# AdrienCorenflos/aux-ssm-samplers

Measured on AMD Instinct MI355X. Metric: Gibbs sweeps/sec (aux-Kalman, parallel-in-time scan), higher is better.
Workload: dtype f64; 1 GPU; C2: linear-Gaussian SSM T=65536 d=4 p=8, aux-Kalman sweep, parallel scan; chains_per_gpu=256, parallelism=chains x1 (independent, no collective)

## Files before the change

### aux_ssm_samplers_amd/csrc/fused_shared.h

```cpp
#pragma once

struct FusedArgs {
    int C, T, E, nchunk;
    const void* xa;
    void* xb;
    const int32_t* sel;
    void* u;
    void* inc;
    const void* gain;
    const void* samp;
    const void* logt;
    const void* gpre;
    const void* m0p;
    void* agg_f; void* pre_f; void* agg_s; void* pre_s;
    Acc* pa;
    Acc* pe;
    void* pell;
    const Acc* clog;
    const int* nanrow;
    unsigned ka0, ka1, ks0, ks1;
    const void* eps0s;
    double delta, shd;
    const double* dptr;
    int nan_policy;
// ... 191 lines not shown
                    sample_offset<R, D>(G[q], acc, e[h + q], o);
#pragma unroll
                    for (int i = 0; i < D; ++i) acc[i] = j == j0 ? e[h + q][i] : o[i];
                }
            }
        }
    }
    R Gs[DD];
    ldmat(gks, 0, Gs);
#pragma unroll
    for (int s = 0; s < FS_MID_STAGES; ++s) {
        const int off = 1 << s;
        R Gn[DD];
        ldmat(gks, s + 1 < FS_MID_STAGES ? s + 1 : s, Gn);
        stv<R, D>(lds + tid * Pre::NPAD, acc);
        __syncthreads();
        R left[D];
        ldv<R, D>(lds + max(tid - off, 0) * Pre::NPAD, left);
        __syncthreads();
        R o[D];
        sample_offset<R, D>(Gs, left, acc, o);
#pragma unroll
        for (int i = 0; i < D; ++i) acc[i] = tid >= off ? o[i] : acc[i];
#pragma unroll
        for (int k = 0; k < DD; ++k) Gs[k] = Gn[k];
    }
    stv<R, D>(lds + tid * Pre::NPAD, acc);
    __syncthreads();
    R p[D];
    ldv<R, D>(lds + max(tid - 1, 0) * Pre::NPAD, p);
#pragma unroll
    for (int i = 0; i < D; ++i) p[i] = tid > 0 ? p[i] : (R)0;
    for (int jb = j0; jb < j1; jb += NR) {
        if (E2 > NR) load_block(jb);
#pragma unroll
        for (int h = 0; h < NR; h += NG) {
            R G[NG][DD];
#pragma unroll
            for (int q = 0; q < NG; ++q) ldmat(gser, min(jb + h + q, jlast) - j0, G[q]);
#pragma unroll
            for (int q = 0; q < NG; ++q) {
                const int j = jb + h + q;
                if (j < j1) {
                    stv<R, D>(pre + (long long)j * Pre::NPAD, p);
                    R o[D];
                    sample_offset<R, D>(G[q], p, e[h + q], o);
#pragma unroll
                    for (int i = 0; i < D; ++i) p[i] = o[i];
                }
            }
        }
    }
}
template <typename R, int D>
__global__ void __launch_bounds__(TB_AGGS) k_fs_mid(FusedArgs a, const R* __restrict__ gtab_f, const R* __restrict__ gtab_s) {
    using Pre = SampPre<R, D>;
    __shared__ __attribute__((aligned(16))) R lds[TB_AGGS * Pre::NPAD];
    const long long base = (long long)blockIdx.x * a.nchunk * Pre::NPAD;
    R* pre_f = (R*)a.pre_f + base;
    const size_t nks = fs_mid_ks_reals<D>(), nser = fs_mid_ser_reals<D>(a.nchunk);
    fs_mid_scan<R, D, false>(lds, a.nchunk, (const R*)a.agg_f + base, pre_f, gtab_f, gtab_f + nks, nullptr, nullptr);
    __syncthreads();
    fs_mid_scan<R, D, true>(lds, a.nchunk, (const R*)a.agg_s + base, (R*)a.pre_s + base, gtab_s, gtab_s + nks, gtab_s + nks + nser, pre_f);
}

template <typename R, int D, int PO> struct FsRows {
    static constexpr int P = D + PO;
    using TL = LogShared<R, D, PO>;
    static constexpr int VEC = 16 / sizeof(R);
    static constexpr int pad(int n) { return (n + VEC - 1) / VEC * VEC; }
    static constexpr int cM = 0, cKc = D * D, cK = cKc + D, cM1 = cK + D * D, cGb = cM1 + D * D, cL = cGb + D, cGp = cL + symsize(D), cLg = cGp + D * D,
                         NC = pad(cLg + TL::N);
    static constexpr int eG = 0, eN = D * D, eL = 2 * D * D, NE = pad(eL + TL::N);
};
struct FsSrc { int tab, off; };
template <typename R, int D, int PO> __device__ __forceinline__ FsSrc fs_src_c(int k) {
    constexpr int P = D + PO;
    using F = FsRows<R, D, PO>; using TG = GainRow<R, D, P>; using TS = SampShared<R, D>; using TL = LogShared<R, D, PO>;
    if (k < F::cKc) return {0, TG::oM + k};
    if (k < F::cK) return {0, TG::oKc + (k - F::cKc)};
    if (k < F::cM1) { const int q = k - F::cK; return {0, TG::oK + (q / D) * P + (q % D)}; }
    if (k < F::cGb) return {1, TS::oM + (k - F::cM1)};
    if (k < F::cL) return {1, TS::oGb + (k - F::cGb)};
    if (k < F::cGp) {
        const int q = k - F::cL;
        int i = 0;
        while (lidx(i + 1, 0) <= q) ++i;
        return {1, TS::oL + i * D + (q - lidx(i, 0))};
    }
    if (k < F::cLg) return {3, k - F::cGp};
    if (k < F::cLg + TL::N) return {2, k - F::cLg};
    return {-1, 0};
}
template <typename R, int D, int PO> __device__ __forceinline__ FsSrc fs_src_e(int k) {
    using F = FsRows<R, D, PO>; using TS = SampShared<R, D>; using TL = LogShared<R, D, PO>;
    if (k < F::eN) return {1, TS::oG + k};
    if (k < F::eL) return {5, k - F::eN};
    if (k < F::eL + TL::N) return {4, k - F::eL};
    return {-1, 0};
}
template <typename R, int D, int PO> __global__ void __launch_bounds__(256) k_fs_rows(FusedArgs a, const R* __restrict__ ntab, R* __restrict__ rc, R* __restrict__ re,
                                                                                      int* __restrict__ nanrow) {
    if (memo_skip(a)) return;
    constexpr int P = D + PO;
    using F = FsRows<R, D, PO>; using TG = GainRow<R, D, P>; using TS = SampShared<R, D>; using TL = LogShared<R, D, PO>;
    const int fam = blockIdx.y;
    const int N = fam == 0 ? F::NC : F::NE;
    const long long g = (long long)blockIdx.x * 256 + threadIdx.x;
    if (g >= (long long)a.T * N) return;
    const int t = (int)(g / N), k = (int)(g % N);
    const FsSrc sc = fam == 0 ? fs_src_c<R, D, PO>(k) : fs_src_e<R, D, PO>(k);
    R v = 0;
    if (sc.tab == 0) { if (t >= 1) v = ((const R*)a.gain)[(long long)(t - 1) * TG::NPAD + sc.off]; }
    else if (sc.tab == 1) v = ((const R*)a.samp)[(long long)t * TS::NPAD + sc.off];
    else if (sc.tab == 2) { if (t >= 1) v = ((const R*)a.logt)[(long long)(t - 1) * TL::NPAD + sc.off]; }
    else if (sc.tab == 3) v = ((const R*)a.gpre)[(long long)t * D * D + sc.off];
    else if (sc.tab == 4) { if (t + 1 < a.T) v = ((const R*)a.logt)[(long long)t * TL::NPAD + sc.off]; }
    else if (sc.tab == 5) v = ntab[(long long)t * D * D + sc.off];
    (fam == 0 ? rc : re)[g] = v;
    if ((sc.tab == 2 || sc.tab == 4) && !finite_(v)) *nanrow = 1;
}

template <typename R, int D> __global__ void __launch_bounds__(256) k_fs_clog_part(int T, const R* __restrict__ samp, Acc* __restrict__ part, const int* memo) {
    if (memo_skip_p(memo)) return;
    using TS = SampShared<R, D>;
    __shared__ Acc sh[256];
    const int t = blockIdx.x * 256 + threadIdx.x;
    R s = 0;
    if (t < T) {
        const R* row = samp + (long long)t * TS::NPAD;
#pragma unroll
        for (int i = 0; i < D; ++i) s += log_(row[TS::oL + i * D + i]);
    }
    sh[threadIdx.x] = (Acc)s;
    __syncthreads();
    for (int off = 128; off > 0; off >>= 1) {
        if ((int)threadIdx.x < off) sh[threadIdx.x] += sh[threadIdx.x + off];
        __syncthreads();
    }
    if (threadIdx.x == 0) part[blockIdx.x] = sh[0];
}
template <int D> __global__ void __launch_bounds__(256) k_fs_clog_sum(int T, int nb, const Acc* __restrict__ part, Acc* __restrict__ out, int* __restrict__ nanrow,
                                                                      const int* memo) {
    if (memo_skip_p(memo)) return;
    if (threadIdx.x == 0) *nanrow = 0;
    __shared__ Acc sh[256];
    Acc acc = 0;
    for (int b = threadIdx.x; b < nb; b += 256) acc += part[b];
    sh[threadIdx.x] = acc;
    __syncthreads();
    for (int off = 128; off > 0; off >>= 1) {
        if ((int)threadIdx.x < off) sh[threadIdx.x] += sh[threadIdx.x + off];
        __syncthreads();
    }
    if (threadIdx.x == 0) *out = sh[0] + (Acc)T * (Acc)D * (Acc)(0.5 * LOG_2PI);
}

__device__ __forceinline__ void fs_block(const FusedArgs& a, int& ch, int& c, bool down = false) {
    const int groups = (a.C + (int)blockDim.x - 1) / (int)blockDim.x;
    const int q = blockIdx.x / groups;
    ch = down ? a.nchunk - 1 - q : q;
    c = (blockIdx.x % groups) * blockDim.x + threadIdx.x;
}
template <typename R, int N> __device__ __forceinline__ void fs_stage(const R* __restrict__ tab, int r0, int r1, R* __restrict__ lds) {
    using V = typename Vec16<R>::type;
    constexpr int W = Vec16<R>::W;
    const V* src = reinterpret_cast<const V*>(tab + (long long)r0 * N);
    V* dst = reinterpret_cast<V*>(lds);
    const int n = (r1 - r0) * (N / W), B = blockDim.x;
    for (int i = threadIdx.x; i < n; i += 4 * B) {
        const bool p1 = i + B < n, p2 = i + 2 * B < n, p3 = i + 3 * B < n;
        const V v0 = src[i], v1 = p1 ? src[i + B] : V{}, v2 = p2 ? src[i + 2 * B] : V{}, v3 = p3 ? src[i + 3 * B] : V{};
        dst[i] = v0;
        if (p1) dst[i + B] = v1;
        if (p2) dst[i + 2 * B] = v2;
        if (p3) dst[i + 3 * B] = v3;
    }
    __syncthreads();
}

template <typename R, int N> __device__ __forceinline__ void fs_stage_pk(const R* __restrict__ tab, int r0, int r1, int E, R* __restrict__ lds) {
    using V = typename Vec16<R>::type;
    constexpr int W = Vec16<R>::W, NV = N / W;
    const V* src = reinterpret_cast<const V*>(tab + (long long)r0 * N);
    V* dst = reinterpret_cast<V*>(lds);
    const int n = (r1 - r0) * NV, B = blockDim.x;
    for (int i = threadIdx.x; i < n; i += 8 * B) {
        V v[8];
#pragma unroll
        for (int q = 0; q < 8; ++q) v[q] = i + q * B < n ? src[i + q * B] : V{};
#pragma unroll
        for (int q = 0; q < 8; ++q)
            if (i + q * B < n) dst[i + q * B + ((i + q * B) / NV) / E] = v[q];
    }
    __syncthreads();
}
template <typename R, int N> AX_HD size_t fs_pk_block(int E) { return (size_t)E * N + Vec16<R>::W; }

template <typename R> struct FsNormTabSel { using type = NormTabGlobal; static constexpr size_t BYTES = 0; };
template <> struct FsNormTabSel<double> { using type = NormTabLds; static constexpr size_t BYTES = (size_t)RNG_TAB_DOUBLES * sizeof(double); };
template <typename R> using FsNormTab = typename FsNormTabSel<R>::type;
template <typename R> __device__ __forceinline__ FsNormTab<R> fs_stage_normtab(R* behind_rows) {
    if constexpr (sizeof(R) == 8) {
        NormTabLds::stage((double*)behind_rows, false);
        return NormTabLds{(const double*)behind_rows};
    } else {
        return NormTabGlobal{};
    }
}

template <typename R, int D, int PO>
__device__ __forceinline__ void fs_terms(const FusedArgs& a, const R* row, const R* v, const R* w, const R* u, R inv_delta, R cst, R* out3) {
    using TL = LogShared<R, D, PO>;
    R ob;
    bool badobs = false;
    {
        R q = 0;
#pragma unroll
        for (int k = 0; k < PO; ++k) {
            R z = row[TL::oYw + k];
#pragma unroll
            for (int j = 0; j < D; ++j) z -= row[TL::oWH + k * D + j] * v[j];
            badobs = badobs || !finite_(z);
            q += z * z;
        }
        ob = (R)-0.5 * q + row[TL::oCR];
        if (badobs || isnan_(ob)) ob = 0;
    }
    asm volatile("" ::: "memory");
    R ax, qa = 0;
    bool b = false;
    {
#pragma unroll
        for (int k = 0; k < D; ++k) {
            const R d = u[k] - v[k];
            b = b || !finite_(d);
            qa += d * d;
        }
        ax = b ? (R)0 : -qa * inv_delta + cst;
    }
    const R cc = (a.nan_policy == 0 && (b || badobs)) ? (R)0 : ax + ob;
    asm volatile("" ::: "memory");
    R pr;
    {
        R q = 0;
        bool bad = false;
#pragma unroll
        for (int k = 0; k < D; ++k) {
            R z = -row[TL::oWb + k];
#pragma unroll
            for (int l = 0; l <= k; ++l) z += row[TL::oWQ + lidx(k, l)] * v[l];
#pragma unroll
            for (int j = 0; j < D; ++j) z -= row[TL::oWF + k * D + j] * w[j];
            bad = bad || !finite_(z);
            q += z * z;
        }
        pr = (R)-0.5 * q + row[TL::oCQ];
        if (bad || isnan_(pr)) pr = 0;
    }
    out3[0] = cc + pr;
    out3[1] = ob + pr;
    out3[2] = qa * inv_delta;
}

template <typename R, int D, int PO>
__device__ __forceinline__ bool fs_terms_fast(const R* row, const R* v, const R* w, const R* u, R inv_delta, R cst, R* out3) {
    using TL = LogShared<R, D, PO>;
    R qo = 0;
#pragma unroll
    for (int k = 0; k < PO; ++k) {
        R z = row[TL::oYw + k];
#pragma unroll
        for (int j = 0; j < D; ++j) z -= row[TL::oWH + k * D + j] * v[j];
        qo += z * z;
    }
    const R ob = (R)-0.5 * qo + row[TL::oCR];
    asm volatile("" ::: "memory");
    R qa = 0;
#pragma unroll
    for (int k = 0; k < D; ++k) {
        const R d = u[k] - v[k];
        qa += d * d;
    }
    const R ax = -qa * inv_delta + cst;
    asm volatile("" ::: "memory");
    R qp = 0;
#pragma unroll
    for (int k = 0; k < D; ++k) {
        R z = -row[TL::oWb + k];
#pragma unroll
        for (int l = 0; l <= k; ++l) z += row[TL::oWQ + lidx(k, l)] * v[l];
#pragma unroll
        for (int j = 0; j < D; ++j) z -= row[TL::oWF + k * D + j] * w[j];
        qp += z * z;
    }
    const R pr = (R)-0.5 * qp + row[TL::oCQ];
    out3[0] = (ax + ob) + pr;
    out3[1] = ob + pr;
    out3[2] = qa * inv_delta;
    return !finite_(out3[0]);
}
__device__ __forceinline__ bool fs_wave_any(bool flag) { return __builtin_amdgcn_ballot_w64(flag) != 0; }

constexpr int FS_WPE_A = 2;
template <typename R, int D, int PO, bool PK = false>
__global__ void __launch_bounds__(256) __attribute__((amdgpu_waves_per_eu(FS_WPE_A))) k_fs_ac(FusedArgs a, const R* __restrict__ rows) {
    using F = FsRows<R, D, PO>;
    extern __shared__ __attribute__((aligned(16))) char smem[];
    R* lds = (R*)smem;
    fs_resolve(a);
    int ch, c;
    if constexpr (PK) {
        const int sub = (int)threadIdx.x / a.cp;
        c = (int)threadIdx.x - sub * a.cp;
        ch = blockIdx.x * a.pack + sub;
    } else {
        fs_block(a, ch, c);
    }
    const long long C = a.C;
    const int t0 = ch * a.E, ta = max(1, t0), tb = min(a.T, t0 + a.E);
    const FsNormTab<R> ntab = fs_stage_normtab<R>(lds + (PK ? (size_t)a.pack * fs_pk_block<R, F::NC>(a.E) : (size_t)a.E * F::NC));
    if constexpr (PK) {
        const int c0 = blockIdx.x * a.pack;
        fs_stage_pk<R, F::NC>(rows, c0 * a.E, min(a.T, (c0 + a.pack) * a.E), a.E, lds);
        lds += (size_t)(ch - c0) * fs_pk_block<R, F::NC>(a.E);
        if (ch >= a.nchunk) return;
    } else {
        fs_stage<R, F::NC>(rows, t0, tb, lds);
    }
    if (c >= a.C) return;
    const R* xr = (const R*)((a.sel && a.sel[c]) ? (const void*)a.xb : a.xa) + c;
    R* up = (R*)a.u + c;
    R* ip = (R*)a.inc + c;
    R h[D], xq[D], es[D];
#pragma unroll
    for (int k = 0; k < D; ++k) {
        h[k] = ch == 0 ? ((const R*)a.m0p)[k * C + c] : (R)0;
        xq[k] = xr[((long long)(ta - 1) * D + k) * C];
        es[k] = 0;
    }
    const R shd = (R)a.shd, inv_delta = (R)1 / (R)a.delta;
    const R cst = (R)-0.5 * (R)D * log_((R)(0.5 * a.delta)) - (R)(0.5 * LOG_2PI) * (R)D;
    Acc v0 = 0, v1 = 0, v2 = 0;
    R se = 0;
    auto emit = [&](int tu, const R* row, const R* eps) {
        R inc[D];
#pragma unroll
        for (int k = 0; k < D; ++k) se += eps[k] * eps[k];
#pragma unroll
        for (int i = 0; i < D; ++i) {
            R v = -row[F::cGb + i];
#pragma unroll
            for (int k = 0; k < D; ++k) v += row[F::cM1 + i * D + k] * h[k];
#pragma unroll
            for (int k = 0; k <= i; ++k) v += row[F::cL + lidx(i, k)] * eps[k];
            inc[i] = v;
            ip[((long long)tu * D + i) * C] = v;
        }
#pragma unroll
        for (int i = 0; i < D; ++i) {
            R v = es[i];
#pragma unroll
            for (int k = 0; k < D; ++k) v += row[F::cGp + i * D + k] * inc[k];
            es[i] = v;
        }
    };
    if (ch == 0) {
        R eps[D];
#pragma unroll
        for (int k = 0; k < D; ++k) eps[k] = ((const R*)a.eps0s)[k * C + c];
        emit(0, lds, eps);
    }
    R xn[D];
#pragma unroll
    for (int k = 0; k < D; ++k) xn[k] = ta < tb ? xr[((long long)ta * D + k) * C] : (R)0;
#pragma unroll 1
    for (int t = ta; t < tb; ++t) {
        const int tu = PK ? t : opaque_uniform(t);
        const R* row = lds + (tu - t0) * F::NC;
        R x[D], ev[D], u[D];
#pragma unroll
        for (int k = 0; k < D; ++k) x[k] = xn[k];
        if (t + 1 < tb) {
            const int tn = PK ? t + 1 : opaque_uniform(t + 1);
#pragma unroll
            for (int k = 0; k < D; ++k) xn[k] = xr[((long long)tn * D + k) * C];
        }
        normals_cm<R, D>(a.ka0, a.ka1, (long long)tu * D * C + c, C, ev, ntab);
#pragma unroll
        for (int k = 0; k < D; ++k) {
            u[k] = x[k] + shd * ev[k];
            up[((long long)tu * D + k) * C] = u[k];
        }
        asm volatile("" ::: "memory");
        R w[3], um[D];
        const bool bad = fs_terms_fast<R, D, PO>(row + F::cLg, x, xq, u, inv_delta, cst, w);
#pragma unroll
        for (int k = 0; k < D; ++k) um[k] = u[k];
        if (fs_wave_any(bad)) {
            fs_terms<R, D, PO>(a, row + F::cLg, x, xq, u, inv_delta, cst, w);
#pragma unroll
            for (int k = 0; k < D; ++k) um[k] = finite_(u[k]) ? u[k] : (R)0;
        }
        v0 += (Acc)w[0];
        v1 += (Acc)w[1];
        v2 += (Acc)w[2];
        asm volatile("" ::: "memory");
        {
            R o[D];
#pragma unroll
            for (int r = 0; r < D; ++r) {
                R v = row[F::cKc + r];
#pragma unroll
                for (int k = 0; k < D; ++k) v += row[F::cM + r * D + k] * h[k];
#pragma unroll
                for (int k = 0; k < D; ++k) v += row[F::cK + r * D + k] * um[k];
                o[r] = v;
            }
#pragma unroll
            for (int r = 0; r < D; ++r) h[r] = o[r];
        }
        asm volatile("" ::: "memory");
        R eps[D];
        normals_cm<R, D>(a.ks0, a.ks1, (long long)tu * D * C + c, C, eps, ntab);
        emit(tu, row, eps);
#pragma unroll
        for (int k = 0; k < D; ++k) xq[k] = x[k];
    }
    stv<R, D>((R*)a.agg_f + ((long long)c * a.nchunk + ch) * SampPre<R, D>::NPAD, h);
    stv<R, D>((R*)a.agg_s + ((long long)c * a.nchunk + (a.nchunk - 1 - ch)) * SampPre<R, D>::NPAD, es);
    a.pa[((long long)0 * C + c) * a.nchunk + ch] = v0;
    a.pa[((long long)1 * C + c) * a.nchunk + ch] = v1;
    a.pa[((long long)2 * C + c) * a.nchunk + ch] = v2;
    ((R*)a.pell)[(long long)c * a.nchunk + ch] = (R)-0.5 * se;
}

template <bool ONCE, typename R> __device__ __forceinline__ R fs_ld_once(const R* p) {
    if constexpr (ONCE) return __builtin_nontemporal_load(p);
    else return *p;
}
template <bool ONCE, typename R> __device__ __forceinline__ void fs_st_once(R* p, R v) {
    if constexpr (ONCE) __builtin_nontemporal_store(v, p);
    else *p = v;
}
template <typename R, int D, int PO, bool PK = false> __global__ void __launch_bounds__(256) k_fs_e(FusedArgs a, const R* __restrict__ rows) {
    using F = FsRows<R, D, PO>;
    extern __shared__ __attribute__((aligned(16))) char smem[];
    R* lds = (R*)smem;
    fs_resolve(a);
    int ch, c;
    if constexpr (PK) {
        const int sub = (int)threadIdx.x / a.cp;
        c = (int)threadIdx.x - sub * a.cp;
        ch = blockIdx.x * a.pack + sub;
    } else {
        fs_block(a, ch, c, true);
    }
    const long long C = a.C;
    const int t0 = ch * a.E, tb = min(a.T, t0 + a.E);
    if constexpr (PK) {
        const int c0 = blockIdx.x * a.pack;
        fs_stage_pk<R, F::NE>(rows, c0 * a.E, min(a.T, (c0 + a.pack) * a.E), a.E, lds);
        lds += (size_t)(ch - c0) * fs_pk_block<R, F::NE>(a.E);
        if (ch >= a.nchunk) return;
    } else {
        fs_stage<R, F::NE>(rows, t0, tb, lds);
    }
    if (c >= a.C) return;
    R* xw = (R*)((a.sel && a.sel[c]) ? const_cast<void*>(a.xa) : a.xb) + c;
    const R* up = (const R*)a.u + c;
    const R* ip = (const R*)a.inc + c;
    R h[D], uq[D], mst[D];
    if (ch > 0) {
        ldv<R, D>((const R*)a.pre_f + ((long long)c * a.nchunk + ch) * SampPre<R, D>::NPAD, mst);
    } else {
#pragma unroll
        for (int k = 0; k < D; ++k) mst[k] = 0;
    }
    if (ch == a.nchunk - 1) {
#pragma unroll
        for (int k = 0; k < D; ++k) h[k] = 0, uq[k] = 0;
    } else {
        ldv<R, D>((const R*)a.pre_s + ((long long)c * a.nchunk + (a.nchunk - 1 - ch)) * SampPre<R, D>::NPAD, h);
#pragma unroll
        for (int k = 0; k < D; ++k) uq[k] = up[((long long)tb * D + k) * C];
    }
    const R inv_delta = (R)1 / (R)a.delta;
    const R cst = (R)-0.5 * (R)D * log_((R)(0.5 * a.delta)) - (R)(0.5 * LOG_2PI) * (R)D;
    Acc v0 = 0, v1 = 0, v2 = 0;
    R incn[D], utn[D];
#pragma unroll
    for (int k = 0; k < D; ++k) incn[k] = fs_ld_once<!PK>(ip + ((long long)(tb - 1) * D + k) * C), utn[k] = fs_ld_once<!PK>(up + ((long long)(tb - 1) * D + k) * C);
#pragma unroll 1
    for (int t = tb - 1; t >= t0; --t) {
        const int tu = PK ? t : opaque_uniform(t);
        const R* row = lds + (tu - t0) * F::NE;
        R inc[D], ut[D], xp[D];
#pragma unroll
        for (int k = 0; k < D; ++k) inc[k] = incn[k], ut[k] = utn[k];
        if (t > t0) {
            const int tn = PK ? t - 1 : opaque_uniform(t - 1);
#pragma unroll
            for (int k = 0; k < D; ++k) incn[k] = fs_ld_once<!PK>(ip + ((long long)tn * D + k) * C), utn[k] = fs_ld_once<!PK>(up + ((long long)tn * D + k) * C);
        }
#pragma unroll
        for (int i = 0; i < D; ++i) {
            R v = inc[i];
#pragma unroll
            for (int k = 0; k < D; ++k) v += row[F::eN + i * D + k] * mst[k];
#pragma unroll
            for (int k = 0; k < D; ++k) v += row[F::eG + i * D + k] * h[k];
            xp[i] = v;
            fs_st_once<!PK>(xw + ((long long)tu * D + i) * C, v);
        }
        if (tu + 1 < a.T) {
            R w[3];
            if (fs_wave_any(fs_terms_fast<R, D, PO>(row + F::eL, h, xp, uq, inv_delta, cst, w))) fs_terms<R, D, PO>(a, row + F::eL, h, xp, uq, inv_delta, cst, w);
            v0 += (Acc)w[0];
            v1 += (Acc)w[1];
            v2 += (Acc)w[2];
        }
#pragma unroll
        for (int k = 0; k < D; ++k) h[k] = xp[k], uq[k] = ut[k];
    }
    a.pe[((long long)0 * C + c) * a.nchunk + ch] = v0;
    a.pe[((long long)1 * C + c) * a.nchunk + ch] = v1;
    a.pe[((long long)2 * C + c) * a.nchunk + ch] = v2;
}

template <typename R, int D, int PO> __global__ void __launch_bounds__(TB_ELEM) k_fs_head(SweepLogpdfArgs la, const void* xa, const void* xb, const int32_t* sel, R* __restrict__ head5) {
    resolve_step(la);
    const int c = blockIdx.x * TB_ELEM + threadIdx.x;
    if (c >= la.d.C) return;
    const bool sw = sel && sel[c];
    la.x.ptr = sw ? xb : xa;
    la.xp.ptr = sw ? xa : xb;
    R h5[5];
    body_sweep_logpdf_head<R, D, PO>(la, c, h5);
#pragma unroll
    for (int k = 0; k < 5; ++k) head5[(long long)k * la.d.C + c] = h5[k];
}

template <typename R, int D, int PO> __device__ __forceinline__ Acc fs_dropped_joint(const FusedArgs& a, const SweepLogpdfArgs& la, int c, const int32_t* sel) {
    Acc s = 0;
    const long long C = a.C;
    const R* xp = (const R*)((sel && sel[c]) ? a.xa : (const void*)a.xb) + c;
    const R* up = (const R*)a.u + c;
    const R inv_delta = (R)1 / (R)a.delta;
    const R cst = (R)-0.5 * (R)D * log_((R)(0.5 * a.delta)) - (R)(0.5 * LOG_2PI) * (R)D;
    for (int t = threadIdx.x; t < a.T; t += TB_ELEM) {
        R y[PO];
        rd<R, PO>(la.ys, c, t, 0, y);
        bool skip[PO], any = false;
#pragma unroll
        for (int k = 0; k < PO; ++k) skip[k] = !finite_(y[k]), any = any || skip[k];
        if (!any) continue;
        R H[PO * D], cv[PO], Rm[PO * PO], v[D], r[PO], q = 0;
        bool b = false;
        rd<R, PO * D>(la.Hs, c, t, 0, H);
        rd<R, PO>(la.cs, c, t, 0, cv);
        rd_upper<R, PO>(la.Rs, c, t, 0, Rm);
#pragma unroll
        for (int k = 0; k < D; ++k) {
            v[k] = xp[((long long)t * D + k) * C];
            const R d = up[((long long)t * D + k) * C] - v[k];
            b = b || !finite_(d);
            q += d * d;
        }
#pragma unroll
        for (int k = 0; k < PO; ++k) {
            R p = cv[k];
#pragma unroll
            for (int j = 0; j < D; ++j) p += H[k * D + j] * v[j];
            r[k] = y[k] - p;
        }
        s += (Acc)(b ? (R)0 : -q * inv_delta + cst) + (Acc)gauss_logpdf<R, PO>(r, Rm, skip);
    }
    return s;
}
template <typename R, int D, int PO> __global__ void __launch_bounds__(TB_ELEM) k_fs_accept(FusedArgs a, SweepLogpdfArgs lg, const R* __restrict__ head5, const R* __restrict__ ell0,
                                                                                            const R* __restrict__ u_acc, int32_t* __restrict__ accepted, R* __restrict__ logs,
                                                                                            int32_t* __restrict__ sel) {
    __shared__ Acc sh[TB_ELEM];
    fs_resolve(a);
    const int c = blockIdx.x;
    const long long C = a.C;
    bool any_dropped = false;
    if (a.nan_policy == 0) {
        R y0[PO];
        rd<R, PO>(lg.ys, c, 0, 0, y0);
        any_dropped = *a.nanrow != 0;
#pragma unroll
        for (int k = 0; k < PO; ++k) any_dropped = any_dropped || !finite_(y0[k]);
    }
    Acc tot[7] = {0, 0, 0, 0, 0, 0, 0};
    const R* pl = (const R*)a.pell + (long long)c * a.nchunk;
    for (int j = threadIdx.x; j < a.nchunk; j += TB_ELEM) {
#pragma unroll
        for (int k = 0; k < 3; ++k) tot[k] += a.pa[((long long)k * C + c) * a.nchunk + j], tot[3 + k] += a.pe[((long long)k * C + c) * a.nchunk + j];
        tot[6] += (Acc)pl[j];
    }
#pragma unroll
    for (int k = 0; k < 7; ++k) tot[k] = block_sum<Acc, TB_ELEM>(tot[k], sh);
    Acc dropped = 0;
    if (any_dropped) dropped = block_sum<Acc, TB_ELEM>(fs_dropped_joint<R, D, PO>(a, lg, c, sel), sh);
    if (threadIdx.x != 0) return;
    (void)ell0;
    const Acc jp_prop = tot[3] + (Acc)head5[0 * C + c], jp_rev = tot[0] + (Acc)head5[1 * C + c];
    const Acc ell = (jp_prop + dropped) - (tot[6] - *a.clog);
    const Acc lt_prop = tot[4] + (Acc)head5[2 * C + c], lt_rev = tot[1] + (Acc)head5[3 * C + c];
    const Acc corr = (tot[5] - tot[2]) + (Acc)head5[4 * C + c];
    const Acc lp_prop = jp_prop - ell, lp_rev = jp_rev - ell;
    Acc la = lt_prop - lt_rev;
    la += lp_rev - lp_prop;
    la -= corr;
    const Acc alpha = exp_(la != la ? la : min_(la, (Acc)0));
    const int acc = ((Acc)u_acc[c] < alpha) ? 1 : 0;
    accepted[c] = acc;
    if (sel) sel[c] ^= acc;
    if (logs) {
        logs[c * 5 + 0] = (R)la;
        logs[c * 5 + 1] = (R)lp_prop;
        logs[c * 5 + 2] = (R)lp_rev;
        logs[c * 5 + 3] = (R)lt_prop;
        logs[c * 5 + 4] = (R)lt_rev;
    }
}

inline int fs_pack(int C, int* cp_out) {
    int cp = 2;
    while (cp < C) cp <<= 1;
    *cp_out = cp;
    constexpr int lanes = 256;
    if (cp > lanes / 2) return 1;
    const int pack = lanes / cp;
    constexpr int cap = 8;
    return pack > cap ? cap : pack;
}
inline int fs_chunk_len(const auxssm_ctx* h, int C, int T) {
    constexpr int waves = 10;
    const long long stiles = (C + TB_CM - 1) / TB_CM;
    long long want = (long long)h->num_cu * 4 * waves / stiles;
    if (want < 1) want = 1;
    long long E = (T + want - 1) / want;
    if (E < 16) E = 16;
    if (E > 32) E = 32;
    if (C >= 1024) E = 64;
    else if (C >= 96) E = 32;
    if (E > T) E = T > 2 ? T : 2;
    return (int)E;
}
template <typename R, int D, int PO> size_t fused_ws(const auxssm_ctx* h, const KDims& d) {
    constexpr int P = D + PO;
    const int E = fs_chunk_len(h, d.C, d.T), nchunk = (d.T + E - 1) / E;
    size_t b = 0;
    b += (size_t)d.C * nchunk * (4 * SampPre<R, D>::NPAD * sizeof(R) + 6 * sizeof(Acc) + sizeof(R)) + 16 * 256;
    b += (size_t)d.C * (5 + 1 + D) * sizeof(R) + 4 * 256;
    b += filter_ws<R, D, P>(h, KDims{1, d.T, 1}, 1);
    b += (size_t)d.T * (SampShared<R, D>::NPAD + LogShared<R, D, PO>::NPAD + (size_t)D * D) * sizeof(R) + (size_t)2 * nchunk * D * D * sizeof(R) + 10 * 256 + ((size_t)d.T / 256 + 2) * sizeof(Acc);
    b += (size_t)d.T * (FsRows<R, D, PO>::NC + FsRows<R, D, PO>::NE + 2 * (size_t)D * D) * sizeof(R) + (size_t)nchunk * D * D * sizeof(R) + 8 * 256;
    b += (2 * fs_mid_ks_reals<D>() + 3 * fs_mid_ser_reals<D>(nchunk)) * sizeof(R) + 2 * 256;
    return b;
}
template <typename R, int D, int PO> int run_fused_shared(auxssm_ctx* h, FusedHost& f) {
    constexpr int P = D + PO;
    const int C = f.fa.d.C, T = f.fa.d.T, n = T - 1;
    FusedArgs a{};
    a.C = C; a.T = T;
    a.E = fs_chunk_len(h, C, T);
    a.nchunk = (T + a.E - 1) / a.E;
    a.pack = fs_pack(C, &a.cp);
    {
        using FR = FsRows<R, D, PO>;
        constexpr int NMAX = FR::NC > FR::NE ? FR::NC : FR::NE;
        while (a.pack > 1 && (size_t)a.pack * fs_pk_block<R, NMAX>(a.E) * sizeof(R) + FsNormTabSel<R>::BYTES > (size_t)128 * 1024) a.pack >>= 1;
    }
    a.xa = f.xa; a.xb = f.xb; a.sel = f.sel; a.u = f.u; a.inc = f.inc;
    a.ka0 = f.keys[0]; a.ka1 = f.keys[1]; a.ks0 = f.keys[2]; a.ks1 = f.keys[3];
    a.eps0s = f.eps0s;
    a.delta = f.la.delta; a.shd = f.la.shd; a.dptr = f.la.dptr; a.nan_policy = f.la.nan_policy;
    a.memo = f.memo;
    f.fa.memo = f.sa.memo = f.la.memo = f.memo;
    R *cprod_f, *cprod_s, *rows_c, *rows_e, *psi, *gtab_f, *gtab_s;
    {
        {
            const int rc = build_gain_table<R, D, P>(h, f.fa);
            if (rc) return rc;
        }
        SideScope side(h);
        f.sa.tab = ws_take(h, (size_t)T * SampShared<R, D>::NPAD * sizeof(R));
        f.la.tab = ws_take(h, (size_t)n * LogShared<R, D, PO>::NPAD * sizeof(R));
        R* gpre = (R*)ws_take(h, (size_t)T * D * D * sizeof(R));
        cprod_f = (R*)ws_take(h, (size_t)a.nchunk * D * D * sizeof(R));
        cprod_s = (R*)ws_take(h, (size_t)a.nchunk * D * D * sizeof(R));
        rows_c = (R*)ws_take(h, (size_t)T * FsRows<R, D, PO>::NC * sizeof(R));
        rows_e = (R*)ws_take(h, (size_t)T * FsRows<R, D, PO>::NE * sizeof(R));
        R* fpre = (R*)ws_take(h, (size_t)T * D * D * sizeof(R));
        R* ntab = (R*)ws_take(h, (size_t)T * D * D * sizeof(R));
        psi = (R*)ws_take(h, (size_t)a.nchunk * D * D * sizeof(R));
        const size_t nks = fs_mid_ks_reals<D>(), nser = fs_mid_ser_reals<D>(a.nchunk);
        gtab_f = (R*)ws_take(h, (nks + nser) * sizeof(R));
        gtab_s = (R*)ws_take(h, (nks + 2 * nser) * sizeof(R));
        const int nclb = (T + 255) / 256;
        Acc* clog = (Acc*)ws_take(h, 256 + (size_t)nclb * sizeof(Acc));
        if (!f.sa.tab || !f.la.tab || !gpre || !cprod_f || !cprod_s || !rows_c || !rows_e || !fpre || !ntab || !psi || !gtab_f || !gtab_s || !clog) return AUXSSM_ERR_NOMEM;
        a.clog = clog;
        int* nanrow = (int*)(clog + 16);
        a.nanrow = nanrow;
        a.gain = f.fa.tab; a.samp = f.sa.tab; a.logt = f.la.tab; a.gpre = gpre;
        {
            ProfScope ps(h, AUXSSM_K_SAMPLE_INIT);
            hipLaunchKernelGGL((k_sample_shared_tab<R, D>), dim3((T + TB_ELEM - 1) / TB_ELEM), dim3(TB_ELEM), 0, h->stream, f.sa);
            hipLaunchKernelGGL((k_fs_clog_part<R, D>), dim3(nclb), dim3(256), 0, h->stream, T, (const R*)f.sa.tab, clog + 32, f.memo);
            hipLaunchKernelGGL((k_fs_clog_sum<D>), dim3(1), dim3(256), 0, h->stream, T, nclb, (const Acc*)(clog + 32), clog, nanrow, f.memo);
            hipLaunchKernelGGL((k_sweep_logpdf_tab<R, D, PO>), dim3((n + TB_ELEM - 1) / TB_ELEM), dim3(TB_ELEM), 0, h->stream, f.la);
            hipLaunchKernelGGL((k_fs_fprod<R, D, P>), dim3((a.nchunk + TB_CM - 1) / TB_CM), dim3(TB_CM), 0, h->stream, a, cprod_f, fpre);
            hipLaunchKernelGGL((k_fs_gpre<R, D>), dim3((a.nchunk + TB_CM - 1) / TB_CM), dim3(TB_CM), 0, h->stream, a, gpre, cprod_s);
            hipLaunchKernelGGL((k_fs_psi<R, D>), dim3((a.nchunk + TB_CM - 1) / TB_CM), dim3(TB_CM), 0, h->stream, a, (const R*)gpre, (const R*)fpre, ntab, psi);
            hipLaunchKernelGGL((k_fs_gtab<R, D>), dim3(1), dim3(TB_AGGS), 0, h->stream, a, (const R*)cprod_f, (const R*)nullptr, gtab_f, gtab_f + nks, (R*)nullptr);
            hipLaunchKernelGGL((k_fs_gtab<R, D>), dim3(1), dim3(TB_AGGS), 0, h->stream, a, (const R*)cprod_s, (const R*)psi, gtab_s, gtab_s + nks, gtab_s + nks + nser);
            {
                using F = FsRows<R, D, PO>;
                const long long nmax = (long long)T * (F::NC > F::NE ? F::NC : F::NE);
                hipLaunchKernelGGL((k_fs_rows<R, D, PO>), dim3((unsigned)((nmax + 255) / 256), 2), dim3(256), 0, h->stream, a, (const R*)ntab, rows_c, rows_e, nanrow);
            }
        }
    }
    {
// ... 55 lines not shown
```

### aux_ssm_samplers_amd/csrc/rng.h

```cpp
#pragma once
#include "smallmat.h"
#include "det_math.h"

namespace ax {

AX_HD uint32_t rotl32(uint32_t x, int r) { return (x << r) | (x >> (32 - r)); }

AX_HD void threefry2x32(uint32_t k0, uint32_t k1, uint32_t& x0, uint32_t& x1) {
    const uint32_t ks[3] = {k0, k1, 0x1BD11BDAu ^ k0 ^ k1};
    constexpr int ROT[8] = {13, 15, 26, 6, 17, 29, 16, 24};
    x0 += ks[0];
    x1 += ks[1];
#pragma unroll
    for (int r = 0; r < 20; ++r) {
        x0 += x1;
        x1 = rotl32(x1, ROT[r % 8]);
        x1 ^= x0;
        if (r % 4 == 3) {
            const int j = r / 4 + 1;
            x0 += ks[j % 3];
            x1 += ks[(j + 1) % 3] + (uint32_t)j;
        }
    }
}

template <typename R> AX_HD R bits_to_uniform(uint32_t b);
template <> AX_HD float bits_to_uniform<float>(uint32_t b) { return (float)(b >> 8) * 5.9604644775390625e-8f; }
template <> AX_HD double bits_to_uniform<double>(uint32_t b) { return (double)b * 2.3283064365386963e-10; }

AX_HD float rng_fma(float a, float b, float c) { return fmaf(a, b, c); }
AX_HD double rng_fma(double a, double b, double c) { return fma(a, b, c); }
template <typename R> struct SinCosPoly;
template <> struct SinCosPoly<float> {
    static constexpr int NS = 4, NC = 4;
    static constexpr float S[4] = {-1.6666667163e-01f, 8.3333337680e-03f, -1.9841270114e-04f, 2.7557314297e-06f};
    static constexpr float Cc[4] = {4.1666667908e-02f, -1.3888889225e-03f, 2.4801587642e-05f, -2.7557314297e-07f};
};
template <> struct SinCosPoly<double> {
    static constexpr int NS = 6, NC = 6;
    static constexpr double S[6] = {-1.66666666666666324348e-01, 8.33333333332248946124e-03, -1.98412698298579493134e-04,
                                    2.75573137070700676789e-06,  -2.50507602534068634195e-08, 1.58969099521155010221e-10};
    static constexpr double Cc[6] = {4.16666666666666019037e-02,  -1.38888888888741095749e-03, 2.48015872894767294178e-05,
                                     -2.75573143513906633035e-07, 2.08757232129817482790e-09,  -1.13596475577881948265e-11};
};
template <typename R> AX_HD void sincos_2pi(R u, R& c, R& s) {
    using P = SinCosPoly<R>;
    const R q = rint((R)4 * u);
    const R f = rng_fma((R)-0.25, q, u);
    const R th = (R)6.283185307179586476925286766559 * f;
    const R z = th * th;
    R ps = P::S[P::NS - 1], pc = P::Cc[P::NC - 1];
#pragma unroll
    for (int k = P::NS - 2; k >= 0; --k) ps = rng_fma(ps, z, P::S[k]);
#pragma unroll
    for (int k = P::NC - 2; k >= 0; --k) pc = rng_fma(pc, z, P::Cc[k]);
    const R sn = rng_fma(th * z, ps, th);
    const R cs = rng_fma(z * z, pc, rng_fma((R)-0.5, z, (R)1));
    const int qi = (int)q & 3;
    const R a = (qi & 1) ? sn : cs, b = (qi & 1) ? cs : sn;
    c = (qi == 1 || qi == 2) ? -a : a;
    s = (qi >= 2) ? -b : b;
}

#include "rng_tables.h"
static const double RNG_LOG_TAB_HOST[2 * 257] = AX_RNG_LOG_TAB_INIT;
static const double RNG_TURN_TAB_HOST[2 * 256] = AX_RNG_TURN_TAB_INIT;
#if defined(__HIPCC__)
static __device__ const double __attribute__((aligned(16))) RNG_LOG_TAB_DEV[2 * 257] = AX_RNG_LOG_TAB_INIT;
static __device__ const double __attribute__((aligned(16))) RNG_TURN_TAB_DEV[2 * 256] = AX_RNG_TURN_TAB_INIT;
#endif
constexpr int RNG_TAB_DOUBLES = 2 * 257 + 2 * 256 + 2;
constexpr int RNG_TAB_TURN_OFF = 2 * 257 + 2;
struct NormTabGlobal {
    AX_HD void log_entry(int j, double& inv, double& L) const {
#if defined(__HIP_DEVICE_COMPILE__)
        const double2 e = reinterpret_cast<const double2*>(RNG_LOG_TAB_DEV)[j];
        inv = e.x, L = e.y;
#else
        inv = RNG_LOG_TAB_HOST[2 * j], L = RNG_LOG_TAB_HOST[2 * j + 1];
#endif
    }
    AX_HD void turn_entry(int j, double& c, double& s) const {
#if defined(__HIP_DEVICE_COMPILE__)
        const double2 e = reinterpret_cast<const double2*>(RNG_TURN_TAB_DEV)[j];
        c = e.x, s = e.y;
#else
        c = RNG_TURN_TAB_HOST[2 * j], s = RNG_TURN_TAB_HOST[2 * j + 1];
#endif
    }
};
#if defined(__HIPCC__)
struct NormTabLds {
    const double* p;
    __device__ __forceinline__ static void stage(double* lds, bool sync = true) {
        const double2* s0 = reinterpret_cast<const double2*>(RNG_LOG_TAB_DEV);
        const double2* s1 = reinterpret_cast<const double2*>(RNG_TURN_TAB_DEV);
        double2* d0 = reinterpret_cast<double2*>(lds);
        double2* d1 = reinterpret_cast<double2*>(lds + RNG_TAB_TURN_OFF);
        const int B = blockDim.x;
        for (int i = threadIdx.x; i < 257; i += 4 * B) {
            const bool p1 = i + B < 257, p2 = i + 2 * B < 257, p3 = i + 3 * B < 257;
            const bool q0 = i < 256, q1 = i + B < 256, q2 = i + 2 * B < 256, q3 = i + 3 * B < 256;
            const double2 z{0, 0};
            const double2 a0 = s0[i], a1 = p1 ? s0[i + B] : z, a2 = p2 ? s0[i + 2 * B] : z, a3 = p3 ? s0[i + 3 * B] : z;
            const double2 b0 = q0 ? s1[i] : z, b1 = q1 ? s1[i + B] : z, b2 = q2 ? s1[i + 2 * B] : z, b3 = q3 ? s1[i + 3 * B] : z;
            d0[i] = a0;
            if (p1) d0[i + B] = a1;
            if (p2) d0[i + 2 * B] = a2;
            if (p3) d0[i + 3 * B] = a3;
            if (q0) d1[i] = b0;
            if (q1) d1[i + B] = b1;
            if (q2) d1[i + 2 * B] = b2;
            if (q3) d1[i + 3 * B] = b3;
        }
        if (sync) __syncthreads();
    }
    __device__ __forceinline__ void log_entry(int j, double& inv, double& L) const {
        const double2 e = reinterpret_cast<const double2*>(p)[j];
        inv = e.x, L = e.y;
    }
    __device__ __forceinline__ void turn_entry(int j, double& c, double& s) const {
        const double2 e = reinterpret_cast<const double2*>(p + RNG_TAB_TURN_OFF)[j];
        c = e.x, s = e.y;
    }
};
#endif
AX_HD double sqrt_pos(double x) {
#if defined(__HIP_DEVICE_COMPILE__)
    const double y = __builtin_amdgcn_rsq(x);
    double g = x * y, h = 0.5 * y;
    const double e = fma(-h, g, 0.5);
    g = fma(g, e, g);
    h = fma(h, e, h);
    const double d = fma(-g, g, x);
    return fma(d, h, g);
#else
    return sqrt(x);
#endif
}
template <typename TAB> AX_HD void bm_fp64(uint32_t b0, uint32_t b1, const TAB& tab, double& z0, double& z1) {
    const double v = (double)b0 + 0.5;
#if defined(__HIP_DEVICE_COMPILE__)
    const double mant = __builtin_amdgcn_frexp_mant(v);
    const int ex = __builtin_amdgcn_frexp_exp(v);
#else
    int ex;
    const double mant = frexp(v, &ex);
#endif
    const double jd = rint(fma(mant, 512.0, -256.0));
    double inv, Lj;
    tab.log_entry((int)jd, inv, Lj);
    const double t = fma(jd, -0.001953125, mant - 0.5) * inv;
    const double dk = (double)(ex - 32);
    double p = fma(t, -0.4, 0.5);
    p = fma(p, t, -0.66666666666666663);
    p = fma(p, t, 1.0);
    double L = fma(dk, AX_RNG_NEG2LN2, Lj);
    L = fma(t, -2.0, L);
    L = fma(p, t * t, L);
    const double r = sqrt_pos(L);
    const int jj = (int)((b1 + 0x800000u) >> 24);
    const int sl = (int)(b1 << 8) >> 8;
    double C, S;
    tab.turn_entry(jj, C, S);
    const double th = fma((double)sl, AX_RNG_TURN_SCALE, 0.5 * AX_RNG_TURN_SCALE);
    const double z = th * th;
    const double sf = fma(th * z, fma(z, 8.3333333333333332e-3, -1.6666666666666666e-1), th);
    double cf = fma(z, -1.3888888888888889e-3, 4.1666666666666664e-2);
    cf = fma(cf, z, -0.5);
    cf = fma(cf, z, 1.0);
    z0 = r * fma(-S, sf, C * cf);
    z1 = r * fma(C, sf, S * cf);
}
template <typename R> AX_HD void bits_to_normal2(uint32_t b0, uint32_t b1, R& z0, R& z1);
template <> AX_HD void bits_to_normal2<double>(uint32_t b0, uint32_t b1, double& z0, double& z1) { bm_fp64(b0, b1, NormTabGlobal{}, z0, z1); }
template <typename R, typename TAB> AX_HD void bits_to_normal2_t(uint32_t b0, uint32_t b1, const TAB& tab, R& z0, R& z1) {
    if constexpr (sizeof(R) == 8) bm_fp64(b0, b1, tab, z0, z1);
    else bits_to_normal2<R>(b0, b1, z0, z1);
}
template <> AX_HD void bits_to_normal2<float>(uint32_t b0, uint32_t b1, float& z0, float& z1) {
    const float u1 = ((float)(b0 >> 8) + 0.5f) * 5.9604644775390625e-8f;
    const float u2 = ((float)(b1 >> 8) + 0.5f) * 5.9604644775390625e-8f;
#if defined(__HIP_DEVICE_COMPILE__)
    const float r = __builtin_amdgcn_sqrtf(-1.3862943611198906f * __builtin_amdgcn_logf(u1));
#else
    const float r = sqrtf(-2.0f * logf(u1));
#endif
    float c, s;
#if defined(__HIP_DEVICE_COMPILE__)
    c = __builtin_amdgcn_cosf(u2);
    s = __builtin_amdgcn_sinf(u2);
#else
    sincos_2pi<float>(u2, c, s);
#endif
    z0 = r * c;
    z1 = r * s;
}
AX_HD void stream_counter(uint32_t stream, unsigned long long blk, uint32_t& x0, uint32_t& x1) {
    x0 = (uint32_t)(blk & 0xffffffffull);
    x1 = stream ^ (uint32_t)((blk >> 32) << 16);
}
template <typename R> AX_HD R stream_normal(uint32_t k0, uint32_t k1, uint32_t stream, unsigned long long idx) {
    uint32_t x0, x1;
    stream_counter(stream, idx >> 1, x0, x1);
    threefry2x32(k0, k1, x0, x1);
    R z0, z1;
    bits_to_normal2<R>(x0, x1, z0, z1);
    return (idx & 1) ? z1 : z0;
}
template <typename R> AX_HD R stream_uniform(uint32_t k0, uint32_t k1, uint32_t stream, unsigned long long idx) {
    uint32_t x0, x1;
    stream_counter(stream, idx >> 1, x0, x1);
    threefry2x32(k0, k1, x0, x1);
    return bits_to_uniform<R>((idx & 1) ? x1 : x0);
}
template <typename R, typename TAB = NormTabGlobal>
AX_HD void stream_normal2(uint32_t k0, uint32_t k1, uint32_t stream, unsigned long long blk, R& z0, R& z1, const TAB& tab = TAB{}) {
    uint32_t x0, x1;
    stream_counter(stream, blk, x0, x1);
    threefry2x32(k0, k1, x0, x1);
    bits_to_normal2_t<R>(x0, x1, tab, z0, z1);
}
template <typename R> AX_HD void stream_uniform2(uint32_t k0, uint32_t k1, uint32_t stream, unsigned long long blk, R& u0, R& u1) {
    uint32_t x0, x1;
    stream_counter(stream, blk, x0, x1);
    threefry2x32(k0, k1, x0, x1);
    u0 = bits_to_uniform<R>(x0);
    u1 = bits_to_uniform<R>(x1);
}


#if defined(__HIP_DEVICE_COMPILE__)
__device__ __forceinline__ float swap_neighbour(float v) { return __int_as_float(__builtin_amdgcn_mov_dpp(__float_as_int(v), 0xB1, 0xF, 0xF, true)); }
__device__ __forceinline__ double swap_neighbour(double v) {
    const int lo = __builtin_amdgcn_mov_dpp(__double2loint(v), 0xB1, 0xF, 0xF, true), hi = __builtin_amdgcn_mov_dpp(__double2hiint(v), 0xB1, 0xF, 0xF, true);
    return __hiloint2double(hi, lo);
}
#endif
template <typename R, int D, typename TAB = NormTabGlobal>
AX_HD void normals_cm(uint32_t k0, uint32_t k1, long long base, long long stride, R* out, const TAB& tab = TAB{}) {
#if defined(__HIP_DEVICE_COMPILE__)
    const bool odd = base & 1;
    const long long be = base - (odd ? 1 : 0);
    const uint32_t quarter = odd ? 0x40000000u : 0u, sgn = odd ? 0x80000000u : 0u;
    auto pair = [&](int kk, R& keep, R& send) {
        uint32_t x0, x1;
        stream_counter(0, (unsigned long long)((be + kk * stride) >> 1), x0, x1);
        threefry2x32(k0, k1, x0, x1);
        if constexpr (sizeof(R) == 8) {
            double kp, sd;
            bm_fp64(x0, x1 - quarter, tab, kp, sd);
            keep = kp;
            send = __hiloint2double(__double2hiint(sd) ^ (int)sgn, __double2loint(sd));
        } else {
            R z0, z1;
            bits_to_normal2<R>(x0, x1, z0, z1);
            keep = odd ? z1 : z0;
            send = odd ? z0 : z1;
        }
    };
#pragma unroll
    for (int k = 0; k + 1 < D; k += 2) {
        R keep, send;
        pair(odd ? k + 1 : k, keep, send);
        const R recv = swap_neighbour(send);
        out[k] = odd ? recv : keep;
        out[k + 1] = odd ? keep : recv;
    }
    if (D & 1) {
        R keep, send;
        pair(D - 1, keep, send);
        out[D - 1] = keep;
    }
#else
#pragma unroll
    for (int k = 0; k < D; ++k) out[k] = stream_normal<R>(k0, k1, 0, (unsigned long long)(base + k * stride));
#endif
}

}
```

Measured before the change: 302,000 sweeps/s.

## Software-pipeline RNG table gathers with LDS row loads via sched barriers

Splits the Box-Muller normal generation into index, table-gather and transform phases, then interleaves these with explicit LDS row loads into registers and the observation/prior log-density terms, separated by scheduling barriers. The intent is to hide LDS and table-lookup latency behind the threefry and matrix arithmetic inside the serial time loop. It also raises the waves-per-EU hint for the non-packed kernel from 2 to 3. In exchange, register pressure rises from holding row slices and RNG blocks, which could cause spills, and the fixed barriers restrict the compiler's own scheduling.

Result: no change. 303,500 sweeps/s, median of 2 (+0.5%).

```diff
diff --git a/aux_ssm_samplers_amd/csrc/fused_shared.h b/aux_ssm_samplers_amd/csrc/fused_shared.h
--- a/aux_ssm_samplers_amd/csrc/fused_shared.h
+++ b/aux_ssm_samplers_amd/csrc/fused_shared.h
@@ -517,9 +517,55 @@
 }
 __device__ __forceinline__ bool fs_wave_any(bool flag) { return __builtin_amdgcn_ballot_w64(flag) != 0; }
 
-constexpr int FS_WPE_A = 2;
+template <int A, int B, typename R> __device__ __forceinline__ void fs_take(const R* row, R* s) {
+#pragma unroll
+    for (int k = 0; k < B - A; ++k) s[k] = row[A + k];
+}
+__device__ __forceinline__ void fs_phase() { __builtin_amdgcn_sched_barrier(0); }
+template <typename R, int D, int PO> __device__ __forceinline__ R fs_obs_fast(const R* go, const R* v) {
+    using TL = LogShared<R, D, PO>;
+    constexpr int o = TL::oCQ;
+    R qo = 0;
+#pragma unroll
+    for (int k = 0; k < PO; ++k) {
+        R z = go[TL::oYw - o + k];
+#pragma unroll
+        for (int j = 0; j < D; ++j) z -= go[TL::oWH - o + k * D + j] * v[j];
+        qo += z * z;
+    }
+    return (R)-0.5 * qo + go[TL::oCR - o];
+}
+template <typename R, int D, int PO> __device__ __forceinline__ R fs_prior_fast(const R* gp, R cq, const R* v, const R* w) {
+    using TL = LogShared<R, D, PO>;
+    R qp = 0;
+#pragma unroll
+    for (int k = 0; k < D; ++k) {
+        R z = -gp[TL::oWb + k];
+#pragma unroll
+        for (int l = 0; l <= k; ++l) z += gp[TL::oWQ + lidx(k, l)] * v[l];
+#pragma unroll
+        for (int j = 0; j < D; ++j) z -= gp[TL::oWF + k * D + j] * w[j];
+        qp += z * z;
+    }
+    return (R)-0.5 * qp + cq;
+}
+template <typename R, int D> __device__ __forceinline__ bool fs_sum_fast(R ob, R pr, const R* v, const R* u, R inv_delta, R cst, R* out3) {
+    R qa = 0;
+#pragma unroll
+    for (int k = 0; k < D; ++k) {
+        const R d = u[k] - v[k];
+        qa += d * d;
+    }
+    const R ax = -qa * inv_delta + cst;
+    out3[0] = (ax + ob) + pr;
+    out3[1] = ob + pr;
+    out3[2] = qa * inv_delta;
+    return !finite_(out3[0]);
+}
+
+constexpr int FS_WPE_A = 3, FS_WPE_A_PK = 2;
 template <typename R, int D, int PO, bool PK = false>
-__global__ void __launch_bounds__(256) __attribute__((amdgpu_waves_per_eu(FS_WPE_A))) k_fs_ac(FusedArgs a, const R* __restrict__ rows) {
+__global__ void __launch_bounds__(256) __attribute__((amdgpu_waves_per_eu(PK ? FS_WPE_A_PK : FS_WPE_A))) k_fs_ac(FusedArgs a, const R* __restrict__ rows) {
     using F = FsRows<R, D, PO>;
     extern __shared__ __attribute__((aligned(16))) char smem[];
     R* lds = (R*)smem;
@@ -558,17 +604,24 @@
     const R cst = (R)-0.5 * (R)D * log_((R)(0.5 * a.delta)) - (R)(0.5 * LOG_2PI) * (R)D;
     Acc v0 = 0, v1 = 0, v2 = 0;
     R se = 0;
-    auto emit = [&](int tu, const R* row, const R* eps) {
-        R inc[D];
+    constexpr int NM = F::cL - F::cM1, NL = F::cLg - F::cL;
+    auto emit_mean = [&](const R* gm, R* inc) {
+#pragma unroll
+        for (int i = 0; i < D; ++i) {
+            R v = -gm[F::cGb - F::cM1 + i];
+#pragma unroll
+            for (int k = 0; k < D; ++k) v += gm[i * D + k] * h[k];
+            inc[i] = v;
+        }
+    };
+    auto emit_noise = [&](int tu, const R* gl, const R* eps, R* inc) {
 #pragma unroll
         for (int k = 0; k < D; ++k) se += eps[k] * eps[k];
 #pragma unroll
         for (int i = 0; i < D; ++i) {
-            R v = -row[F::cGb + i];
-#pragma unroll
-            for (int k = 0; k < D; ++k) v += row[F::cM1 + i * D + k] * h[k];
-#pragma unroll
-            for (int k = 0; k <= i; ++k) v += row[F::cL + lidx(i, k)] * eps[k];
+            R v = inc[i];
+#pragma unroll
+            for (int k = 0; k <= i; ++k) v += gl[lidx(i, k)] * eps[k];
             inc[i] = v;
             ip[((long long)tu * D + i) * C] = v;
         }
@@ -576,24 +629,30 @@
         for (int i = 0; i < D; ++i) {
             R v = es[i];
 #pragma unroll
-            for (int k = 0; k < D; ++k) v += row[F::cGp + i * D + k] * inc[k];
+            for (int k = 0; k < D; ++k) v += gl[F::cGp - F::cL + i * D + k] * inc[k];
             es[i] = v;
         }
     };
     if (ch == 0) {
-        R eps[D];
+        R eps[D], inc[D], gm[NM], gl[NL];
 #pragma unroll
         for (int k = 0; k < D; ++k) eps[k] = ((const R*)a.eps0s)[k * C + c];
-        emit(0, lds, eps);
+        fs_take<F::cM1, F::cL>(lds, gm);
+        fs_take<F::cL, F::cLg>(lds, gl);
+        emit_mean(gm, inc);
+        emit_noise(0, gl, eps, inc);
     }
     R xn[D];
 #pragma unroll
     for (int k = 0; k < D; ++k) xn[k] = ta < tb ? xr[((long long)ta * D + k) * C] : (R)0;
+    using NG = NormalsCm<R, D, FsNormTab<R>>;
+    using TL = LogShared<R, D, PO>;
+    constexpr int NB = NG::NB;
 #pragma unroll 1
     for (int t = ta; t < tb; ++t) {
         const int tu = PK ? t : opaque_uniform(t);
         const R* row = lds + (tu - t0) * F::NC;
-        R x[D], ev[D], u[D];
+        R x[D], ev[D], u[D], eps[D];
 #pragma unroll
         for (int k = 0; k < D; ++k) x[k] = xn[k];
         if (t + 1 < tb) {
@@ -601,15 +660,37 @@
 #pragma unroll
             for (int k = 0; k < D; ++k) xn[k] = xr[((long long)tn * D + k) * C];
         }
-        normals_cm<R, D>(a.ka0, a.ka1, (long long)tu * D * C + c, C, ev, ntab);
+        const NG ga(a.ka0, a.ka1, (long long)tu * D * C + c, C, ntab), gs(a.ks0, a.ks1, (long long)tu * D * C + c, C, ntab);
+        typename NG::Blk qa0, qa1, qs0, qs1;
+        R go[TL::N - TL::oCQ], gp[TL::oCQ > 0 ? TL::oCQ : 1];
+        fs_take<F::cLg + TL::oCQ, F::cLg + TL::N>(row, go);
+        fs_phase();
+        ga.bits(0, qa0);
+        fs_phase();
+        ga.gather(qa0);
+        fs_phase();
+        const R ob = fs_obs_fast<R, D, PO>(go, x);
+        const R cq = go[0];
+        fs_phase();
+        fs_take<F::cLg, F::cLg + TL::oCQ>(row, gp);
+        fs_phase();
+        if constexpr (NB > 1) {
+            ga.bits(1, qa1);
+            fs_phase();
+            ga.gather(qa1);
+            fs_phase();
+        }
+        const R pr = fs_prior_fast<R, D, PO>(gp, cq, x, xq);
+        fs_phase();
+        ga.finish(0, qa0, ev);
+        if constexpr (NB > 1) ga.finish(1, qa1, ev);
 #pragma unroll
         for (int k = 0; k < D; ++k) {
             u[k] = x[k] + shd * ev[k];
             up[((long long)tu * D + k) * C] = u[k];
         }
-        asm volatile("" ::: "memory");
         R w[3], um[D];
-        const bool bad = fs_terms_fast<R, D, PO>(row + F::cLg, x, xq, u, inv_delta, cst, w);
+        const bool bad = fs_sum_fast<R, D>(ob, pr, x, u, inv_delta, cst, w);
 #pragma unroll
         for (int k = 0; k < D; ++k) um[k] = u[k];
         if (fs_wave_any(bad)) {
@@ -620,25 +701,45 @@
         v0 += (Acc)w[0];
         v1 += (Acc)w[1];
         v2 += (Acc)w[2];
-        asm volatile("" ::: "memory");
+        fs_phase();
+        R gf[F::cM1], gm[NM], gl[NL], inc[D];
+        fs_take<F::cM, F::cM1>(row, gf);
+        fs_phase();
+        gs.bits(0, qs0);
+        fs_phase();
+        gs.gather(qs0);
+        fs_phase();
         {
             R o[D];
 #pragma unroll
             for (int r = 0; r < D; ++r) {
-                R v = row[F::cKc + r];
-#pragma unroll
-                for (int k = 0; k < D; ++k) v += row[F::cM + r * D + k] * h[k];
-#pragma unroll
-                for (int k = 0; k < D; ++k) v += row[F::cK + r * D + k] * um[k];
+                R v = gf[F::cKc + r];
+#pragma unroll
+                for (int k = 0; k < D; ++k) v += gf[F::cM + r * D + k] * h[k];
+#pragma unroll
+                for (int k = 0; k < D; ++k) v += gf[F::cK + r * D + k] * um[k];
                 o[r] = v;
             }
 #pragma unroll
             for (int r = 0; r < D; ++r) h[r] = o[r];
         }
-        asm volatile("" ::: "memory");
-        R eps[D];
-        normals_cm<R, D>(a.ks0, a.ks1, (long long)tu * D * C + c, C, eps, ntab);
-        emit(tu, row, eps);
+        fs_phase();
+        fs_take<F::cM1, F::cL>(row, gm);
+        fs_phase();
+        if constexpr (NB > 1) {
+            gs.bits(1, qs1);
+            fs_phase();
+            gs.gather(qs1);
+            fs_phase();
+        }
+        emit_mean(gm, inc);
+        fs_phase();
+        fs_take<F::cL, F::cLg>(row, gl);
+        fs_phase();
+        gs.finish(0, qs0, eps);
+        if constexpr (NB > 1) gs.finish(1, qs1, eps);
+        fs_phase();
+        emit_noise(tu, gl, eps, inc);
 #pragma unroll
         for (int k = 0; k < D; ++k) xq[k] = x[k];
     }
diff --git a/aux_ssm_samplers_amd/csrc/rng.h b/aux_ssm_samplers_amd/csrc/rng.h
--- a/aux_ssm_samplers_amd/csrc/rng.h
+++ b/aux_ssm_samplers_amd/csrc/rng.h
@@ -138,19 +138,34 @@
     return sqrt(x);
 #endif
 }
-template <typename TAB> AX_HD void bm_fp64(uint32_t b0, uint32_t b1, const TAB& tab, double& z0, double& z1) {
+struct BmIdx { double dm; int ex, j, jj, sl; };
+struct BmEnt { double inv, Lj, C, S; };
+AX_HD BmIdx bm_fp64_index(uint32_t b0, uint32_t b1) {
+    BmIdx ix;
     const double v = (double)b0 + 0.5;
 #if defined(__HIP_DEVICE_COMPILE__)
     const double mant = __builtin_amdgcn_frexp_mant(v);
-    const int ex = __builtin_amdgcn_frexp_exp(v);
-#else
-    int ex;
-    const double mant = frexp(v, &ex);
+    ix.ex = __builtin_amdgcn_frexp_exp(v);
+#else
+    const double mant = frexp(v, &ix.ex);
 #endif
     const double jd = rint(fma(mant, 512.0, -256.0));
-    double inv, Lj;
-    tab.log_entry((int)jd, inv, Lj);
-    const double t = fma(jd, -0.001953125, mant - 0.5) * inv;
+    ix.j = (int)jd;
+    ix.dm = fma(jd, -0.001953125, mant - 0.5);
+    ix.jj = (int)((b1 + 0x800000u) >> 24);
+    ix.sl = (int)(b1 << 8) >> 8;
+    return ix;
+}
+template <typename TAB> AX_HD BmEnt bm_fp64_gather(const BmIdx& ix, const TAB& tab) {
+    BmEnt en;
+    tab.log_entry(ix.j, en.inv, en.Lj);
+    tab.turn_entry(ix.jj, en.C, en.S);
+    return en;
+}
+AX_HD void bm_fp64_transform(const BmIdx& ix, const BmEnt& en, double& z0, double& z1) {
+    const double inv = en.inv, Lj = en.Lj, C = en.C, S = en.S;
+    const int ex = ix.ex, sl = ix.sl;
+    const double t = ix.dm * inv;
     const double dk = (double)(ex - 32);
     double p = fma(t, -0.4, 0.5);
     p = fma(p, t, -0.66666666666666663);
@@ -159,10 +174,6 @@
     L = fma(t, -2.0, L);
     L = fma(p, t * t, L);
     const double r = sqrt_pos(L);
-    const int jj = (int)((b1 + 0x800000u) >> 24);
-    const int sl = (int)(b1 << 8) >> 8;
-    double C, S;
-    tab.turn_entry(jj, C, S);
     const double th = fma((double)sl, AX_RNG_TURN_SCALE, 0.5 * AX_RNG_TURN_SCALE);
     const double z = th * th;
     const double sf = fma(th * z, fma(z, 8.3333333333333332e-3, -1.6666666666666666e-1), th);
@@ -172,6 +183,10 @@
     z0 = r * fma(-S, sf, C * cf);
     z1 = r * fma(C, sf, S * cf);
 }
+template <typename TAB> AX_HD void bm_fp64(uint32_t b0, uint32_t b1, const TAB& tab, double& z0, double& z1) {
+    const BmIdx ix = bm_fp64_index(b0, b1);
+    bm_fp64_transform(ix, bm_fp64_gather(ix, tab), z0, z1);
+}
 template <typename R> AX_HD void bits_to_normal2(uint32_t b0, uint32_t b1, R& z0, R& z1);
 template <> AX_HD void bits_to_normal2<double>(uint32_t b0, uint32_t b1, double& z0, double& z1) { bm_fp64(b0, b1, NormTabGlobal{}, z0, z1); }
 template <typename R, typename TAB> AX_HD void bits_to_normal2_t(uint32_t b0, uint32_t b1, const TAB& tab, R& z0, R& z1) {
@@ -237,40 +252,63 @@
     return __hiloint2double(hi, lo);
 }
 #endif
-template <typename R, int D, typename TAB = NormTabGlobal>
-AX_HD void normals_cm(uint32_t k0, uint32_t k1, long long base, long long stride, R* out, const TAB& tab = TAB{}) {
-#if defined(__HIP_DEVICE_COMPILE__)
-    const bool odd = base & 1;
-    const long long be = base - (odd ? 1 : 0);
-    const uint32_t quarter = odd ? 0x40000000u : 0u, sgn = odd ? 0x80000000u : 0u;
-    auto pair = [&](int kk, R& keep, R& send) {
-        uint32_t x0, x1;
-        stream_counter(0, (unsigned long long)((be + kk * stride) >> 1), x0, x1);
-        threefry2x32(k0, k1, x0, x1);
+#if defined(__HIPCC__)
+template <typename R, int D, typename TAB> struct NormalsCm {
+    static constexpr int NB = (D + 1) / 2;
+    struct Blk { uint32_t x0, x1; BmIdx ix; BmEnt en; };
+    uint32_t k0, k1, quarter, sgn;
+    long long be, stride;
+    bool odd;
+    const TAB& tab;
+    __device__ __forceinline__ NormalsCm(uint32_t k0_, uint32_t k1_, long long base, long long stride_, const TAB& tab_) : k0(k0_), k1(k1_), stride(stride_), tab(tab_) {
+        odd = base & 1;
+        be = base - (odd ? 1 : 0);
+        quarter = odd ? 0x40000000u : 0u, sgn = odd ? 0x80000000u : 0u;
+    }
+    __device__ __forceinline__ int comp(int b) const { return 2 * b + 1 < D ? (odd ? 2 * b + 1 : 2 * b) : D - 1; }
+    __device__ __forceinline__ void bits(int b, Blk& q) const {
+        stream_counter(0, (unsigned long long)((be + comp(b) * stride) >> 1), q.x0, q.x1);
+        threefry2x32(k0, k1, q.x0, q.x1);
+        if constexpr (sizeof(R) == 8) q.ix = bm_fp64_index(q.x0, q.x1 - quarter);
+    }
+    __device__ __forceinline__ void gather(Blk& q) const {
+        if constexpr (sizeof(R) == 8) q.en = bm_fp64_gather(q.ix, tab);
+    }
+    __device__ __forceinline__ void finish(int b, const Blk& q, R* out) const {
+#if defined(__HIP_DEVICE_COMPILE__)
+        R keep, send;
         if constexpr (sizeof(R) == 8) {
             double kp, sd;
-            bm_fp64(x0, x1 - quarter, tab, kp, sd);
+            bm_fp64_transform(q.ix, q.en, kp, sd);
             keep = kp;
             send = __hiloint2double(__double2hiint(sd) ^ (int)sgn, __double2loint(sd));
         } else {
             R z0, z1;
-            bits_to_normal2<R>(x0, x1, z0, z1);
+            bits_to_normal2<R>(q.x0, q.x1, z0, z1);
             keep = odd ? z1 : z0;
             send = odd ? z0 : z1;
         }
-    };
-#pragma unroll
-    for (int k = 0; k + 1 < D; k += 2) {
-        R keep, send;
-        pair(odd ? k + 1 : k, keep, send);
-        const R recv = swap_neighbour(send);
-        out[k] = odd ? recv : keep;
-        out[k + 1] = odd ? keep : recv;
-    }
-    if (D & 1) {
-        R keep, send;
-        pair(D - 1, keep, send);
-        out[D - 1] = keep;
+        if (2 * b + 1 < D) {
+            const R recv = swap_neighbour(send);
+            out[2 * b] = odd ? recv : keep;
+            out[2 * b + 1] = odd ? keep : recv;
+        } else {
+            out[D - 1] = keep;
+        }
+#endif
+    }
+};
+#endif
+template <typename R, int D, typename TAB = NormTabGlobal>
+AX_HD void normals_cm(uint32_t k0, uint32_t k1, long long base, long long stride, R* out, const TAB& tab = TAB{}) {
+#if defined(__HIP_DEVICE_COMPILE__)
+    const NormalsCm<R, D, TAB> g(k0, k1, base, stride, tab);
+#pragma unroll
+    for (int b = 0; b < g.NB; ++b) {
+        typename NormalsCm<R, D, TAB>::Blk q;
+        g.bits(b, q);
+        g.gather(q);
+        g.finish(b, q, out);
     }
 #else
 #pragma unroll
```
